# ManuelZ/image-search-engine

Measured on AMD Instinct MI355X. Metric: queries/sec, exact brute-force L2 kNN (recall@10 vs exact CPU), 1Mx512 fp32 index, k=10, higher is better.
Workload: dtype f32; 1 GPU; 1000000x512 fp32 uniform[0,1) index (default_rng 1234), L2, k=10, nq=16 queries per step, index resident in HBM, steps issued round-robin on 16 HIP streams; 400 untimed steps ahead of the warm-up bring the GPU out of its idle power state; n=1000000, d=512, k=10, nq=16

## Files before the change

image-search-engine_amd/_native.py:

```python
from __future__ import annotations

import ctypes
import os

import torch

_HERE = os.path.dirname(os.path.abspath(__file__))
LIB_PATH = os.environ.get("ISE_KNN_LIB") or os.path.join(_HERE, "csrc", "libise_knn.so")

METRIC_INNER_PRODUCT = 0
METRIC_L2 = 1
MAX_K = 2048
STORE_F32, STORE_BF16 = 0, 1

E_INVALID, E_HIP, E_NOMEM, E_NODEVICE = -1, -2, -3, -4

_f32p = ctypes.POINTER(ctypes.c_float)
_i64p = ctypes.POINTER(ctypes.c_int64)
_u64p = ctypes.POINTER(ctypes.c_uint64)
_vp = ctypes.c_void_p
_i64 = ctypes.c_int64
_int = ctypes.c_int
PROTOTYPES = [
    ("ise_version", _int, []),
# ... 13 lines not shown
    ("ise_index_add_host", _int, [_vp, _vp, _i64]),
    ("ise_index_add_device", _int, [_vp, _vp, _i64, _vp]),
    ("ise_index_reconstruct_host", _int, [_vp, _i64, _i64, _vp]),
    ("ise_index_search_host", _int, [_vp, _vp, _i64, _int, _vp, _vp]),
    ("ise_index_search_device", _int, [_vp, _vp, _i64, _int, _vp, _vp, _vp]),
    ("ise_index_search_keys_device", _int, [_vp, _vp, _i64, _int, ctypes.c_uint32, _vp, _vp]),
    ("ise_index_assign_device", _int, [_vp, _vp, _i64, _vp, _vp, _vp]),
    ("ise_merge_keys_device", _int, [_vp, _int, _i64, _int, _int, _vp, _vp, _int, _vp]),
    ("ise_normalize_rows_device", _int, [_vp, _i64, _int, _int, _vp]),
    ("ise_normalize_rows_host", _int, [_vp, _i64, _int, _int]),
    ("ise_bovw_histogram_device", _int, [_vp, _vp, _i64, _int, _vp, _int, _vp]),
    ("ise_index_short_stats", _int, [_vp, _vp]),
    ("ise_index_half_stats", _int, [_vp, _u64p]),
    ("ise_index_shadow_row", _int, [_vp, _i64, _f32p]),
    ("ise_index_byte_stats", _int, [_vp, _u64p]),
    ("ise_index_byte_row", _int, [_vp, _i64, _f32p]),
    ("ise_index_stage_query_debug", _int, [_vp, _vp, _int, _vp, _i64, _f32p, ctypes.POINTER(ctypes.c_int32)]),
    ("ise_index_range_search_host", _int, [_vp, _vp, _i64, ctypes.c_float, ctypes.POINTER(_vp)]),
    ("ise_range_result_get", _int, [_vp, _i64p, ctypes.POINTER(_vp), ctypes.POINTER(_vp), ctypes.POINTER(_vp)]),
    ("ise_range_result_destroy", _int, [_vp]),
    ("ise_index_range_stats", _int, [_vp, _u64p]),
    ("ise_index_remove_ids_host", _int, [_vp, _vp, _i64, _i64p]),
    ("ise_index_remove_range", _int, [_vp, _i64, _i64, _i64p]),
    ("ise_index_remove_stats", _int, [_vp, _u64p]),
    ("ise_index_remove_last_timing", _int, [_vp, _f32p, _u64p]),
    ("ise_selector_create_range", _int, [_vp, _i64, _i64, ctypes.POINTER(_vp)]),
    ("ise_selector_create_ids", _int, [_vp, _vp, _i64, _int, ctypes.POINTER(_vp)]),
    ("ise_selector_create_bitmap", _int, [_vp, _vp, _i64, ctypes.POINTER(_vp)]),
    ("ise_selector_info", _int, [_vp, _i64p]),
    ("ise_selector_destroy", _int, [_vp]),
# ... 69 lines not shown
```

image-search-engine_amd/csrc/ise_knn.hip:

```cpp

#include "ise_common.hpp"
#include "ise_scan_params.hpp"
#include "ise_assign.hpp"
#include "ise_exact.hpp"
#include "ise_merge.hpp"
#include "ise_exact_scan.hpp"
#include "ise_gemm_scan.hpp"
#include "ise_gemm_bf16.hpp"
#include "ise_rows.hpp"
#include "ise_short_scan.hpp"
#include "ise_range.hpp"
#include "ise_sel_scan.hpp"
#include "ise_stage.hpp"
#include "ise_remove.hpp"

static thread_local std::string g_err;
static int fail(int code, const std::string& msg) {
    g_err = msg;
    return code;
}
int ise_fail_(int code, const std::string& msg) { return fail(code, msg); }
#define HIP_TRY(expr)                                                                      \
    do {                                                                                   \
        hipError_t e_ = (expr);                                                            \
// ... 12 lines not shown
    bool shift_pinned = false;
    long long mu_rows = 0;
    long long norms_rows = 0;
    void* xh = nullptr;
    float* hmeta = nullptr;
    int dph = 0;
    bool shadow_off = false;
    void* xq8 = nullptr;
    uint32_t* bmeta = nullptr;
    int dpb = 0;
    bool byte_off = false;
    double byte_rel = 0.0;
    double byte_rho = 1.0;
    unsigned long long half_batches = 0;
    unsigned long long byte_batches = 0;
    unsigned long long* stats_dev = nullptr;
    unsigned long long mu_updates = 0;
    unsigned long long gemm_chunks = 0;
    struct WorkSlot {
        u64* part = nullptr;
        size_t part_elems = 0;
        u64* keys_tmp = nullptr;
        size_t keys_tmp_elems = 0;
        u64* xchg = nullptr;
        size_t xchg_elems = 0;
        uint32_t xchg_seq = 0;
        char* gemm = nullptr;
        size_t gemm_bytes = 0;
        u64* fl_state = nullptr;
        int* fl_list = nullptr;
// ... 627 lines not shown
    else if (uses_shift(h)) ise_launch_short_f32_shift(ch, waves, bpc, grid, lds, st, sp, tp);
    else ise_launch_short_f32_plain(ch, waves, bpc, grid, lds, st, sp, tp);
}

struct ScanPlan {
    int nblocks, tiles_total, tiles_per_block, nqt, ch, kpass, kb, waves, T;
    size_t lds;
    bool exact;
    int kc;
    bool gemm;
    size_t gemm_bytes;
    bool half;
    bool byte;
    bool short_;
    int short_bpc;
};

static void launch_scan(const ise_index* h, const ScanPlan& pl, dim3 grid, hipStream_t st, const ScanParams& sp) {
    const int ch = pl.ch, waves = pl.waves, T = pl.T;
    const size_t lds = pl.lds;
    if (pl.byte) ise_launch_scan_i8_shadow(ch, waves, T, grid, lds, st, sp);
    else if (pl.half) ise_launch_scan_f16_shadow(ch, waves, T, grid, lds, st, sp);
    else if (h->storage == ISE_STORE_BF16) ise_launch_scan_bf16(ch, waves, T, grid, lds, st, sp);
    else if (uses_shift(h)) ise_launch_scan_f32_shift(ch, waves, T, grid, lds, st, sp);
    else ise_launch_scan_f32_plain(ch, waves, T, grid, lds, st, sp);
}

static int exact_extra(int k) {
    static const int forced = [] { const char* e = getenv("ISE_EXACT_EXTRA"); return e ? atoi(e) : 0; }();
    (void)k;
// ... 2 lines not shown
static float exact_beta(const ise_index* h) { return (0.5625f * h->dp + 256.f) * 5.9604645e-8f * 1.02f; }
static float half_beta(const ise_index* h) { return (5.f * h->dph + 128.f) * 5.9604645e-8f * 1.02f; }
static float half_lo_shrink(const ise_index* h) { return 1.f - ((float)h->dp / 16.f + 96.f) * 5.9604645e-8f; }
static float byte_beta(const ise_index* h) { return ((float)h->dp / 8.f + 64.f) * 5.9604645e-8f * 1.02f; }
struct EnvKnobs {
    std::atomic<int> force_exact{0};
    std::atomic<int> no_direct{0};
    std::atomic<int> no_short{0};
    std::atomic<int> short_tpb_max{0};
    std::atomic<int> direct_short_max_tiles{0};
    std::atomic<int> range_stage_cap{0};
    std::atomic<int> no_half{0};
    std::atomic<int> no_byte{0};
    std::atomic<int> fail_byte_alloc{0};
    std::atomic<int> remove_slab_rows{0};
    void refresh() {
        auto flag = [](const char* name) { const char* e = getenv(name); return (e && e[0] == '1') ? 1 : 0; };
        auto num = [](const char* name) { const char* e = getenv(name); return e ? atoi(e) : 0; };
        force_exact.store(flag("ISE_FORCE_EXACT"));
        no_direct.store(flag("ISE_NO_DIRECT"));
        no_short.store(flag("ISE_NO_SHORT"));
        short_tpb_max.store(num("ISE_SHORT_TPB_MAX"));
        direct_short_max_tiles.store(num("ISE_DIRECT_SHORT_MAX_TILES"));
        range_stage_cap.store(num("ISE_RANGE_STAGE_CAP"));
        no_half.store(flag("ISE_NO_HALF_FILTER"));
        no_byte.store(flag("ISE_NO_BYTE_FILTER"));
        fail_byte_alloc.store(flag("ISE_FAIL_BYTE_ALLOC"));
        remove_slab_rows.store(num("ISE_REMOVE_SLAB_ROWS"));
    }
};
static EnvKnobs& knobs() {
    static EnvKnobs k;
    static std::once_flag once;
    std::call_once(once, [] { k.refresh(); });
    return k;
}
extern "C" int ise_refresh_env_knobs(void) {
    knobs().refresh();
    return ISE_OK;
}
int ise_remove_slab_rows_() { return knobs().remove_slab_rows.load(std::memory_order_relaxed); }
static bool force_exact() { return knobs().force_exact.load(std::memory_order_relaxed) != 0; }
static bool byte_alloc_refused() { return knobs().fail_byte_alloc.load(std::memory_order_relaxed) != 0; }

static bool xchg_enabled() {
    static const bool on = [] { const char* e = getenv("ISE_NO_XCHG"); return !(e && e[0] == '1'); }();
    return on;
}

static int make_plan(const ise_index* h, long long nq, int k, ScanPlan* pl, bool allow_short = true,
                     bool allow_half = true) {
    pl->exact = uses_shift(h);
    const bool shadow_ok = allow_half && pl->exact && h->xh != nullptr && !knobs().no_half.load(std::memory_order_relaxed);
    pl->byte = shadow_ok && h->xq8 != nullptr && byte_rel_ok(h) && !knobs().no_byte.load(std::memory_order_relaxed) &&
               k <= BYTE_MAX_K && nq <= BYTE_MAX_NQ;
    pl->kc = pl->exact ? (pl->byte ? BYTE_KC : k + exact_extra(k)) : k;
    pl->kpass = pl->kc < KPASS_MAX ? pl->kc : KPASS_MAX;
    pl->kb = pl->kpass <= 16 ? 16 : (pl->kpass <= 32 ? 32 : KB_MAX);
    pl->half = shadow_ok && (pl->byte || pl->kc <= SHADOW_MAX_KC);
    const size_t rb = pl->byte ? byte_row_bytes(h) : (pl->half ? shadow_row_bytes(h) : row_bytes(h));
    auto lds_bytes = [&](int waves, int T) {
        if (pl->byte) return scan_lds_layout(qs_stride_byte(h), waves, T, pl->kb, true, scan_seeded_boot(true, waves, T));
        return pl->half ? scan_lds_layout(qs_stride_half(h), waves, T, pl->kb, true) : scan_lds_bytes(h, waves, T, pl->kb);
    };
    pl->ch = chunk_steps_rb(rb);
#ifdef ISE_ABLATE
// ... 27 lines not shown
        if (!wv) break;
        const double cost = (double)((nq + 16 * t - 1) / (16 * t)) * pass_cost[t];
        if (!pl->T || cost < best - 1e-9) {
            pl->T = t;
            pl->waves = wv;
            pl->lds = lds;
            best = cost;
        }
    }
    if (!pl->T) return fail(ISE_E_INVALID, "d too large: a 16-query tile must fit the 160 KiB LDS "
                                              "(float32 rows: d <= 2240, bf16 rows: d <= 4480)");
    if ((pl->T == 1 || pl->waves == 16) && pl->ch > 4) pl->ch = 4;
    pl->tiles_total = (int)((h->n + 15) / 16);
    int blocks_per_cu = (pl->T == 1 && pl->waves <= 8 && pl->lds <= LDS_LIMIT / 2) ? 2 : 1;
#ifdef ISE_ABLATE
    if (const char* e = getenv("ISE_PLAN")) {
        int wv = 8, bpc = 2;
        if (pl->T == 1 && sscanf(e, "%d,%d", &wv, &bpc) == 2 && (wv == 4 || wv == 8) && bpc >= 1) {
            pl->waves = wv;
            pl->lds = lds_bytes(wv, 1);
            blocks_per_cu = bpc;
        }
    }
#endif
    const bool long_rows = rb > 2048;
    const int nqt_plan = (int)((nq + 16 * pl->T - 1) / (16 * pl->T));
    const int min_tiles = (int)std::max<size_t>(1, 65536 / (16 * rb));
    const int slots = h->num_cu * blocks_per_cu;
    const int nb_packed = std::min(slots, (pl->tiles_total + pl->waves - 1) / pl->waves);
    const int nb_spread = std::min(std::max(1, slots / nqt_plan), (pl->tiles_total + min_tiles - 1) / min_tiles);
    int nb = std::max(nb_packed, nb_spread);
    if (nb < 1) nb = 1;
    if (nb > MERGE_LISTS_MAX) nb = MERGE_LISTS_MAX;
    pl->tiles_per_block = (pl->tiles_total + nb - 1) / nb;
    if (pl->tiles_per_block < 1) pl->tiles_per_block = 1;
    pl->nblocks = (pl->tiles_total + pl->tiles_per_block - 1) / pl->tiles_per_block;
    if (pl->nblocks < 1) pl->nblocks = 1;
    if (long_rows && pl->T == 1 && pl->waves <= 8 && pl->tiles_per_block <= pl->waves && chunk_steps_rb(rb) == 8) pl->ch = 8;
    pl->nqt = (int)((nq + 16 * pl->T - 1) / (16 * pl->T));
    pl->gemm = false;
    pl->gemm_bytes = 0;
    pl->short_ = false;
    pl->short_bpc = 0;
    static const bool short_t2 = [] { const char* e = getenv("ISE_SHORT_T2"); return !(e && e[0] == '0'); }();
    const int short_T = nq <= 16 ? 1 : 2;
    if (allow_short && !pl->byte && (nq <= 16 || (short_t2 && nq <= 64)) && pl->kc <= pl->kpass && h->n > 0 &&
        !knobs().no_short.load(std::memory_order_relaxed)) {
        int tpb_max = knobs().short_tpb_max.load(std::memory_order_relaxed);
        if (tpb_max <= 0 || tpb_max > SHORT_TPB_MAX) tpb_max = SHORT_TPB_MAX;
        const int S = qs_stride_for(h);
        static const int shapes[2][3] = {{16, 1, 1}, {8, 2, 1}};
        int first = row_bytes(h) <= 2048 ? 0 : 2;
#ifdef ISE_ABLATE
        if (const char* e = getenv("ISE_SHORT_SHAPE")) first = std::max(first, std::min(1, atoi(e)));
#endif
        for (int si = first; si < 2 && !pl->short_; si++) {
            const int wv = shapes[si][0], bpc = shapes[si][1];
            const int short_nqt = (int)((nq + 16 * short_T - 1) / (16 * short_T));
            const int packed = (pl->tiles_total + wv - 1) / wv;
            const int spread = std::min(std::max(1, h->num_cu * bpc / short_nqt), (pl->tiles_total + min_tiles - 1) / min_tiles);
            int nbs = std::max(1, std::min(h->num_cu * bpc * shapes[si][2], std::max(packed, spread)));
            nbs = std::min(nbs, MERGE_LISTS_MAX);
            const int tpb = (pl->tiles_total + nbs - 1) / nbs;
            const size_t lds = short_lds_layout(S, tpb, wv, short_T);
            if (tpb <= tpb_max && lds <= (size_t)LDS_LIMIT / bpc) {
                pl->short_ = true;
                pl->nblocks = nbs;
                pl->tiles_per_block = tpb;
                pl->lds = lds;
                pl->waves = wv;
                pl->short_bpc = bpc;
                pl->T = short_T;
                pl->nqt = short_nqt;
                pl->ch = std::min(chunk_steps(h), 4);
                pl->half = false;
                pl->byte = false;
            }
        }
    }
    return ISE_OK;
}

static int ensure_workspace(ise_index::WorkSlot* w, const ScanPlan& pl, long long nq, bool* changed) {
    if (!w->done) HIP_TRY(hipEventCreateWithFlags(&w->done, hipEventDisableTiming));
    const size_t need = std::max<size_t>((size_t)pl.nqt * pl.nblocks * (16 * pl.T) * pl.kpass, (size_t)MERGE_LISTS_MAX * XPASS_MAX);
    if (need > w->part_elems) {
        if (w->part) (void)hipFree(w->part);
        w->part = nullptr;
        w->part_elems = 0;
        HIP_TRY(hipMalloc(&w->part, need * sizeof(u64)));
        w->part_elems = need;
        *changed = true;
    }
    const size_t needx = (size_t)pl.nqt * (16 * pl.T) * pl.nblocks;
    if (needx > w->xchg_elems) {
        if (w->xchg) (void)hipFree(w->xchg);
        w->xchg = nullptr;
        w->xchg_elems = 0;
        HIP_TRY(hipMalloc(&w->xchg, needx * sizeof(u64)));
        HIP_TRY(hipMemset(w->xchg, 0xFF, needx * sizeof(u64)));
        w->xchg_elems = needx;
        w->xchg_seq = 0;
        if (const char* e = getenv("ISE_XCHG_SEQ_START"))
            w->xchg_seq = (uint32_t)strtoul(e, nullptr, 0);
        *changed = true;
    }
    if (pl.kc > pl.kpass) {
        const size_t need2 = (size_t)nq * ((size_t)pl.kc + 2 + pl.kpass + XPASS_MAX);
        if (need2 > w->keys_tmp_elems) {
// ... 89 lines not shown
    *seq = ++w->fl_seq;
    return ISE_OK;
}

template <bool RERANK>
static void launch_merge(unsigned grid, size_t lds, hipStream_t st, const MergeParams& mp, const ExactParams& xp) {
    hipLaunchKernelGGL((merge_kernel<RERANK>), dim3(grid), dim3(MERGE_THREADS), lds, st, mp, xp);
}

static int enqueue_exact_fallback(ise_index* h, ise_index::WorkSlot* w, const ScanPlan& pl, const ExactParams& xp,
                                  long long nq, hipStream_t st) {
    ExactScanParams xs;
    xs.xb = (const float*)h->xb; xs.q = xp.q; xs.n = h->n; xs.d = h->d; xs.dp = h->dp;
    xs.id_base = xp.id_base; xs.fl_state = w->fl_state; xs.fl_list = w->fl_list; xs.seq = xp.seq;
    xs.part = w->part;
    xs.rows_per_block = (long long)pl.tiles_per_block * 16;
    xs.arrive = reinterpret_cast<unsigned int*>(w->fl_state + 1);
    xs.direct_n = 0;
    const size_t lds = (size_t)XQ * h->dp * 4 + (size_t)XQ * 4 * 32 * 8;
    MergeParams mp;
    mp.lists = w->part; mp.qt = 1; mp.n_lists = pl.nblocks; mp.nq = (int)nq; mp.metric = h->metric;
    mp.fl_state = w->fl_state; mp.fl_list = w->fl_list; mp.seq = xp.seq; mp.dbg = nullptr; mp.gate = nullptr;
    const int k = xp.k;
    if (k <= XPASS_MAX) {
        xs.kpass = k; xs.floor_keys = nullptr;
        mp.k = k; mp.stride_list = k; mp.stride_qtile = (long long)pl.nblocks * k;
        mp.D = xp.D; mp.I = xp.I; mp.keys_out = xp.keys_out; mp.out_by_pos = 0;
        hipLaunchKernelGGL(exact_scan_kernel<XQ>, dim3((unsigned)pl.nblocks), dim3(256), lds, st, xs, mp);
        HIP_TRY(hipGetLastError());
        return ISE_OK;
    }
    u64* fb_floor = w->keys_tmp + (size_t)nq * ((size_t)pl.kc + 1 + pl.kpass);
    u64* fb_pass = fb_floor + nq;
    const int kp = XPASS_MAX;
    for (int off = 0; off < k; off += kp) {
        xs.kpass = kp; xs.floor_keys = off ? fb_floor : nullptr;
        mp.k = kp; mp.stride_list = kp; mp.stride_qtile = (long long)pl.nblocks * kp;
        mp.D = nullptr; mp.I = nullptr; mp.keys_out = fb_pass; mp.out_by_pos = 1;
        hipLaunchKernelGGL(exact_scan_kernel<XQ>, dim3((unsigned)pl.nblocks), dim3(256), lds, st, xs, mp);
        const long long tot = nq * kp;
        hipLaunchKernelGGL(exact_scatter_kernel, dim3((unsigned)((tot + 255) / 256)), dim3(256), 0, st, xp,
                           (const u64*)fb_pass, kp, off, fb_floor);
        HIP_TRY(hipGetLastError());
    }
    return ISE_OK;
}

static bool no_direct() { return knobs().no_direct.load(std::memory_order_relaxed) != 0; }
static bool direct_applies(const ise_index* h, const ise_index::WorkSlot* w, const ScanPlan& pl, long long nq, int k,
                           int* blocks_out) {
    if (!pl.exact || nq != 1 || k > XPASS_MAX || h->n <= 0 || !w->fl_state || no_direct() || force_exact()) return false;
    int max_tiles = knobs().direct_short_max_tiles.load(std::memory_order_relaxed);
    if (max_tiles <= 0) max_tiles = 128;
    if (pl.short_ && pl.tiles_total > max_tiles) return false;
// ... 55 lines not shown
    GemmLayout g;
    size_t o = 0;
    auto take = [&](size_t bytes) { const size_t at = o; o += (bytes + 255) / 256 * 256; return at; };
    g.qprep = take((size_t)GEMM_NQ_MAX * qs_stride_for(h) * 4);
    g.xn = take((size_t)GEMM_NQ_MAX * 4);
    g.tau = take((size_t)GEMM_NQ_MAX * 4);
    g.ccnt = take((size_t)(GEMM_NQ_MAX * GEMM_SUBS + 64) * 4);
    g.dump = take((size_t)GEMM_NQ_MAX * GEMM_SAMPLE_SLABS * 128 * 4);
    g.cand = take((size_t)GEMM_NQ_MAX * GEMM_CAPQ * 8);
    g.wbuf = take((size_t)h->num_cu * 8 * GEMM_CAPW * 16);
    g.wcnt = take((size_t)h->num_cu * 8 * 4);
    g.total = o;
    return g;
}

static int plan_for_batch(const ise_index* h, long long nq, int k, ScanPlan* pl) {
    const bool big = gemm_applies(h, nq, k);
    int rc = make_plan(h, big ? std::min<long long>(nq, GEMM_NQ_MAX) : nq, k, pl);
    if (rc) return rc;
    pl->gemm = big;
    pl->gemm_bytes = big ? gemm_layout(h).total : 0;
    return ISE_OK;
}

template <int NS, bool DUMP, bool IPM>
static void launch_gemm_metric(int grid, size_t lds, hipStream_t st, const GemmScanParams& gp) {
    static LdsAttrOnce attr;
    attr.ensure(reinterpret_cast<const void*>(&gemm_scan_kernel<NS, DUMP, IPM>), LDS_LIMIT);
    hipLaunchKernelGGL((gemm_scan_kernel<NS, DUMP, IPM>), dim3(grid), dim3(512), lds, st, gp);
}
template <int NS, bool DUMP>
static void launch_gemm_one(int grid, size_t lds, hipStream_t st, const GemmScanParams& gp) {
    if (gp.metric == ISE_METRIC_INNER_PRODUCT) launch_gemm_metric<NS, DUMP, true>(grid, lds, st, gp);
// ... 86 lines not shown
                             int k, uint32_t id_base, float* D_dev, long long* I_dev, u64* keys_out, hipStream_t st,
                             TimedOut* tm, const unsigned int* gate) {
    int rc;
    ScanParams sp;
    sp.xb = h->xb; sp.norms = h->norms; sp.q = q_dev; sp.mu = h->mu; sp.floor_keys = nullptr; sp.part = w->part;
    sp.n = h->n; sp.d = h->d; sp.dp = h->dp; sp.qs_stride = qs_stride_for(h);
    sp.row_slots = (int)(row_bytes(h) / 16);
    sp.nq = (int)nq; sp.k = pl.kpass; sp.kb = pl.kb; sp.metric = h->metric; sp.id_base = id_base;
    sp.beta = pl.exact ? exact_beta(h) : 0.f;
    if (pl.byte) {
        sp.xb = h->xq8; sp.bmeta = h->bmeta;
        sp.qs_stride = qs_stride_byte(h); sp.row_slots = (int)(byte_row_bytes(h) / 16);
        sp.beta = byte_beta(h); sp.lo_shrink = half_lo_shrink(h);
        h->half_batches++;
        h->byte_batches++;
    } else if (pl.half) {
        sp.xb = h->xh; sp.norms = h->hmeta; sp.herr = h->hmeta + h->cap; sp.hexp = h->hmeta + 2 * h->cap;
        sp.qs_stride = qs_stride_half(h); sp.row_slots = (int)(shadow_row_bytes(h) / 16);
        sp.beta = half_beta(h); sp.lo_shrink = half_lo_shrink(h);
        h->half_batches++;
    }
    sp.tiles_total = pl.tiles_total; sp.tiles_per_block = pl.tiles_per_block;
    sp.xchg = xchg_enabled() ? w->xchg : nullptr;
    sp.xchg_seq = 0;
    sp.gate = gate;
    sp.ablate = 0;
    sp.stamps = nullptr;
#ifdef ISE_ABLATE
    if (const char* e = getenv("ISE_ABLATE")) sp.ablate = atoi(e);
    if (const char* e = getenv("ISE_STAMPS")) sp.stamps = (unsigned long long*)strtoull(e, nullptr, 0);
// ... 246 lines not shown
                       keys_out);
    HIP_TRY(hipGetLastError());
    ScanPlan pl;
    rc = make_plan(h, nq, k, &pl, false);
    if (rc) return rc;
    rc = scan_path_enqueue(h, w, pl, q_dev, nq, k, id_base, D_dev, I_dev, keys_out, st, nullptr, rerun);
    if (rc) return rc;
    if (tm && tm->on) HIP_TRY(hipEventRecord(tm->e2, st));
    return ISE_OK;
}

static int search_enqueue(ise_index* h, const float* q_dev, long long nq, int k, uint32_t id_base, float* D_dev,
                          long long* I_dev, u64* keys_out, hipStream_t st, TimedOut* tm) {
    int rc = prepare_shift_locked(h, st);
    if (rc) return rc;
    ScanPlan pl;
    rc = plan_for_batch(h, nq, k, &pl);
    if (rc) return rc;
    rc = ensure_workspaces(h, pl, pl.gemm ? std::min<long long>(nq, GEMM_NQ_MAX) : nq);
    if (rc) return rc;
    ise_index::WorkSlot* w = nullptr;
    bool same_stream = false;
    for (auto& s : h->ws)
        if (s.used && s.last_stream == st) { w = &s; same_stream = true; break; }
    if (!w)
        for (auto& s : h->ws)
            if (!s.used) { w = &s; break; }
    if (!w) w = &h->ws[h->ws_next++ % ise_index::NWS];
    if (w->used && !same_stream) HIP_TRY(hipStreamWaitEvent(st, w->done, 0));
    struct Release {
        ise_index::WorkSlot* w;
        hipStream_t st;
// ... 1047 lines not shown
extern "C" int ise_index_range_stats(ise_index_t* h, uint64_t* out2) {
    if (!h || !out2) return fail(ISE_E_INVALID, "NULL argument");
    std::lock_guard<std::mutex> lk(h->rg_mu);
    out2[0] = h->range_batches;
    out2[1] = h->range_overflows;
    return ISE_OK;
}

extern "C" int ise_index_short_stats(ise_index_t* h, uint64_t* out1) {
    if (!h || !out1) return fail(ISE_E_INVALID, "NULL argument");
    std::lock_guard<std::mutex> lk(h->mu_);
    out1[0] = h->short_batches;
    return ISE_OK;
}

extern "C" int ise_index_half_stats(ise_index_t* h, uint64_t* out1) {
    if (!h || !out1) return fail(ISE_E_INVALID, "NULL argument");
    std::lock_guard<std::mutex> lk(h->mu_);
    out1[0] = h->half_batches;
    return ISE_OK;
}

extern "C" int ise_index_byte_stats(ise_index_t* h, uint64_t* out2) {
    if (!h || !out2) return fail(ISE_E_INVALID, "NULL argument");
    std::lock_guard<std::mutex> lk(h->mu_);
    out2[0] = h->byte_batches;
    out2[1] = (h->xq8 && byte_rel_ok(h)) ? 1 : 0;
    return ISE_OK;
}

// ... 253 lines not shown
```

image-search-engine_amd/csrc/ise_scan.hpp:

```cpp
#pragma once
#include "ise_common.hpp"
#include "ise_scan_params.hpp"
#include "ise_select.hpp"
#include "ise_stage.hpp"

#ifndef ISE_FINAL_FILTER
#define ISE_FINAL_FILTER 1
#endif

#ifdef ISE_ABLATE
#define ABL(bit) (p.ablate & (bit))
#define STAMP(i)                                                                                   \
    do {                                                                                           \
        if (p.stamps && lane == 0)                                                                 \
            p.stamps[((size_t)blockIdx.x * W + w) * 16 + (i)] = __builtin_amdgcn_s_memrealtime();  \
    } while (0)
#define CSTAMP(i)                                                                                  \
    do {                                                                                           \
        if (p.stamps && lane == 0)                                                                 \
            p.stamps[((size_t)blockIdx.x * W + w) * 16 + (i)] = __builtin_amdgcn_s_memtime();      \
    } while (0)
#else
#define ABL(bit) 0
#define STAMP(i) do {} while (0)
#define CSTAMP(i) do {} while (0)
#endif

template <int CH, int W, int T, bool BF16, bool SHIFT, int RM = ROWS_OWN>
__global__ __launch_bounds__(W * 64, T == 1 ? W / 2 : (W / 4 > 0 ? W / 4 : 1)) void scan_kernel(const ScanParams p) {
    constexpr bool HALF = RM == ROWS_F16, BYTE = RM == ROWS_I8, SHADOW = HALF || BYTE;
    static_assert(!(BF16 && SHIFT), "the shift is applied to fp32 rows only");
    static_assert(!SHADOW || SHIFT, "shadow rows belong to float32 L2 indexes");
    constexpr bool F32S = SHIFT && !SHADOW;
    if (p.gate && *p.gate == 0u) return;
    constexpr int BLOCK_THREADS = W * 64;
    constexpr bool XCHG = T >= 3 || (T == 2 && W == 8) || (RM == ROWS_I8 && T == 1 && W == 8);
    constexpr bool FFILT = XCHG && ISE_FINAL_FILTER;
    constexpr bool NBOOT = scan_seeded_boot(RM == ROWS_I8, W, T);
    static_assert(!NBOOT || XCHG, "the seeded boot reads the exchange");
    constexpr int NQ = 16 * T;
    constexpr int TPR = W >= 16 ? 32 : BLOCK_THREADS / 16;
    constexpr int KPLB = (W * 16 + 63) / 64;
    constexpr int KPLF = (KB_MAX + W * CAP + 63) / 64;
    static_assert(KB_MAX + CAP <= 64 && MERGE_TRIG + 4 <= CAP, "list sizes");
    extern __shared__ __align__(16) unsigned char smem[];
    const int S = p.qs_stride;
    const int kb = p.kb;
    float* mus = reinterpret_cast<float*>(smem);
    float* qs = mus + S;
    float* xn = qs + NQ * S;
    float* xe = xn + NQ;
    int* xsh = reinterpret_cast<int*>(xe + NQ);
    u64* tauS = reinterpret_cast<u64*>(xn + (SHADOW ? 3 : 1) * NQ);
// ... 465 lines not shown
        for (int b = 31; b >= 0; b--) {
            const uint32_t hm = b == 31 ? 0u : 0xFFFFFFFFu << (b + 1);
            auto zero_here = [&](uint32_t v) { return ((v ^ prefix) & hm) == 0u && ((v >> b) & 1u) == 0u; };
            const int c0 = __popcll(__ballot(zero_here(v0))) + __popcll(__ballot(zero_here(v1))) +
                           __popcll(__ballot(zero_here(v2))) + __popcll(__ballot(zero_here(v3)));
            if (rank > c0) {
                rank -= c0;
                prefix |= 1u << b;
            }
        }
        return prefix;
    };
    constexpr bool XFOLD = NBOOT;
    constexpr int XE = 4;
    constexpr int XGRID = 512;
    auto xchg_request = [&](int qq, int half, u64(&e)[XE]) {
        const int nb = (int)gridDim.x;
        const int G = (nb + 255) >> 8;
        const u64* src = p.xchg + ((size_t)blockIdx.y * NQ + qq) * nb;
#pragma unroll
        for (int i = 0; i < XE; i++) {
            const int idx = (lane + 64 * (2 * half + (i >> 1))) * G + (i & 1);
            e[i] = __hip_atomic_load(src + (((i & 1) < G && idx < nb) ? idx : 0), __ATOMIC_RELAXED, __HIP_MEMORY_SCOPE_AGENT);
        }
    };
    auto xchg_fold = [&](int half, const u64(&e)[XE], uint32_t best) -> uint32_t {
        const int nb = (int)gridDim.x;
        const int G = (nb + 255) >> 8;
#pragma unroll
        for (int i = 0; i < XE; i++) {
            const int idx = (lane + 64 * (2 * half + (i >> 1))) * G + (i & 1);
            if ((i & 1) < G && idx < nb && (uint32_t)(e[i] >> 32) == p.xchg_seq) best = min(best, (uint32_t)e[i]);
        }
        return best;
    };
    auto lanes_kth = [&](uint32_t v) -> uint32_t {
        uint32_t prefix = 0;
        int rank = k;
        for (int b = 31; b >= 0; b--) {
            const uint32_t hm = b == 31 ? 0u : 0xFFFFFFFFu << (b + 1);
            const int c0 = __popcll(__ballot(((v ^ prefix) & hm) == 0u && ((v >> b) & 1u) == 0u));
            if (rank > c0) {
                rank -= c0;
                prefix |= 1u << b;
            }
        }
        return prefix;
    };
    auto exchange = [&]() {
        STAMP(12);
        for (int qq = w; qq < NQ; qq += W) {
            uint32_t prefix;
            if (XFOLD && (int)gridDim.x <= XGRID && !ABL(16384)) {
                u64 e[XE];
                xchg_request(qq, 0, e);
                const uint32_t b0 = xchg_fold(0, e, 0xFFFFFFFFu);
                xchg_request(qq, 1, e);
                prefix = lanes_kth(xchg_fold(1, e, b0));
            } else {
                prefix = xchg_prefix(qq);
            }
            if (prefix != 0xFFFFFFFFu) {
                const u64 bound = ((u64)prefix << 32) | 0xFFFFFFFFull;
                if (FFILT && lane == (qq - w) / W) xbound = bound;
                if (lane == 0) {
                    while (atomicCAS(&lockS[qq], 0, 1) != 0) __builtin_amdgcn_s_sleep(1);
                }
                wave_lds_fence();
                if (lane == 0 && bound < tauS[qq]) tauS[qq] = bound;
                wave_lds_fence();
                if (lane == 0) atomicExch(&lockS[qq], 0);
            }
        }
// ... 1 lines not shown
    };

    auto seed_phase = [&]() {
        STAMP(10);
        u64 xe_[XE];
        xchg_request(w, 0, xe_);
        __syncthreads();
        STAMP(11);
        const u64 lt_mask = (1ull << lane) - 1ull;
        for (int qq = w; qq < NQ; qq += W) {
            u64 kk[4];
#pragma unroll
            for (int e = 0; e < 4; e++)
                kk[e] = ((e < 2 ? boot : home2) + (size_t)qq * (W * 16))[lane + 64 * (e & 1)];
            uint32_t folded = xchg_fold(0, xe_, 0xFFFFFFFFu);
            xchg_request(qq, 1, xe_);
            folded = xchg_fold(1, xe_, folded);
            if (qq + W < NQ) xchg_request(qq + W, 0, xe_);
            const uint32_t prefix = lanes_kth(folded);
            if (qq == w) STAMP(12);
            const u64 bound = ((u64)prefix << 32) | 0xFFFFFFFFull;
            if (FFILT && prefix != 0xFFFFFFFFu && lane == (qq - w) / W) xbound = bound;
            u64 keep[4];
            int n_in = 0;
#pragma unroll
            for (int e = 0; e < 4; e++) {
                keep[e] = __ballot(kk[e] <= bound && kk[e] != KEY_PAD);
                n_in += __popcll(keep[e]);
            }
            if (prefix != 0xFFFFFFFFu && n_in <= kb) {
                int off = 0;
#pragma unroll
                for (int e = 0; e < 4; e++) {
                    if ((keep[e] >> lane) & 1ull) bootw[qq * kb + off + __popcll(keep[e] & lt_mask)] = kk[e];
// ... 165 lines not shown
```

image-search-engine_amd/csrc/ise_scan_launch.hpp:

```cpp
#pragma once
#include "ise_scan.hpp"

template <int CH, int W, int T, bool BF16, bool SHIFT, int RM>
static void launch_one(dim3 grid, size_t lds, hipStream_t st, const ScanParams& sp) {
    static LdsAttrOnce attr;
    attr.ensure(reinterpret_cast<const void*>(&scan_kernel<CH, W, T, BF16, SHIFT, RM>), LDS_LIMIT);
    hipLaunchKernelGGL((scan_kernel<CH, W, T, BF16, SHIFT, RM>), grid, dim3(W * 64), lds, st, sp);
}
template <int W, int T, bool BF16, bool SHIFT, int RM>
static void launch_scan_ch(int ch, dim3 grid, size_t lds, hipStream_t st, const ScanParams& sp) {
    switch (ch) {
        case 8:
            if constexpr (W < 16) launch_one<8, W, T, BF16, SHIFT, RM>(grid, lds, st, sp);
            else launch_one<4, W, T, BF16, SHIFT, RM>(grid, lds, st, sp);
            break;
        case 4: launch_one<4, W, T, BF16, SHIFT, RM>(grid, lds, st, sp); break;
        case 2: launch_one<2, W, T, BF16, SHIFT, RM>(grid, lds, st, sp); break;
        default: launch_one<1, W, T, BF16, SHIFT, RM>(grid, lds, st, sp); break;
    }
}
template <bool BF16, bool SHIFT, int RM = ROWS_OWN>
static void launch_scan_v(int ch, int waves, int T, dim3 grid, size_t lds, hipStream_t st, const ScanParams& sp) {
    if constexpr (RM == ROWS_I8) {
        if (waves == 4) launch_scan_ch<4, 1, BF16, SHIFT, RM>(ch, grid, lds, st, sp);
        else launch_scan_ch<8, 1, BF16, SHIFT, RM>(ch, grid, lds, st, sp);
    } else if (T == 1 && waves == 4) launch_scan_ch<4, 1, BF16, SHIFT, RM>(ch, grid, lds, st, sp);
    else if (T == 1) launch_scan_ch<8, 1, BF16, SHIFT, RM>(ch, grid, lds, st, sp);
    else if (T == 2 && waves == 16) launch_scan_ch<16, 2, BF16, SHIFT, RM>(ch, grid, lds, st, sp);
    else if (T == 2) launch_scan_ch<8, 2, BF16, SHIFT, RM>(ch, grid, lds, st, sp);
    else if (T == 3) launch_scan_ch<8, 3, BF16, SHIFT, RM>(ch, grid, lds, st, sp);
    else if constexpr (BF16) launch_scan_ch<8, 4, true, false, ROWS_OWN>(ch, grid, lds, st, sp);
}
```

image-search-engine_amd/csrc/ise_scan_params.hpp:

```cpp
#pragma once
#include "ise_common.hpp"

enum RowMode : int { ROWS_OWN = 0, ROWS_F16 = 1, ROWS_I8 = 2 };

struct ScanParams {
    const void* xb;
    const float* norms;
    const float* herr = nullptr;
    const float* hexp = nullptr;
    const uint32_t* bmeta = nullptr;
    const float* q;
    const float* mu;
    const u64* floor_keys;
    u64* part;
    long long n;
    int d, dp, qs_stride;
    int row_slots;
    int nq, k, kb, metric;
    uint32_t id_base;
    float beta;
    float lo_shrink = 1.f;
    int tiles_total, tiles_per_block;
    unsigned long long* xchg;
    uint32_t xchg_seq;
// ... 31 lines not shown
```

image-search-engine_amd/faiss_compat.py:

```python
from __future__ import annotations

import ctypes
import struct
import threading

import numpy as np

from . import _native as _n

METRIC_INNER_PRODUCT = _n.METRIC_INNER_PRODUCT
METRIC_L2 = _n.METRIC_L2

_FLT_MAX = float(np.finfo(np.float32).max)


def _as_rows(x, d=None) -> np.ndarray:
    x = np.ascontiguousarray(np.asarray(x), dtype=np.float32)
    assert x.ndim == 2, "expected a 2-D array"
    if d is not None:
        assert x.shape[1] == d, f"dimension mismatch: got {x.shape[1]}, index has d={d}"
    return x


def _default_device() -> int:
# ... 214 lines not shown

    def short_stats(self) -> dict:
        out = (ctypes.c_uint64 * 1)()
        _n.check(_n.lib.ise_index_short_stats(self._h, out))
        return {"short_batches": int(out[0])}

    def half_stats(self) -> dict:
        out = (ctypes.c_uint64 * 1)()
        _n.check(_n.lib.ise_index_half_stats(self._h, out))
        return {"half_batches": int(out[0])}

    def byte_stats(self) -> dict:
        out = (ctypes.c_uint64 * 2)()
        _n.check(_n.lib.ise_index_byte_stats(self._h, out))
        return {"byte_batches": int(out[0]), "byte_route": bool(out[1])}

    def byte_row(self, i: int) -> tuple:
        out = (ctypes.c_float * 2)()
        _n.check(_n.lib.ise_index_byte_row(self._h, int(i), out))
        return float(out[0]), float(out[1])

    def shadow_row(self, i: int) -> tuple:
        out = (ctypes.c_float * 3)()
        _n.check(_n.lib.ise_index_shadow_row(self._h, int(i), out))
        return float(out[0]), float(out[1]), int(out[2])

    def stage_query_debug(self, q: "torch.Tensor", route: str) -> dict:
        import torch
        assert q.is_cuda and q.dtype == torch.float32 and q.dim() == 1 and q.is_contiguous() and q.numel() == self.d
        es = {"half": 2, "byte": 1}[route]
# ... 829 lines not shown
```

include/ise_knn.h:

```cpp
#ifndef ISE_KNN_H
#define ISE_KNN_H

#include <stdint.h>

#ifdef __cplusplus
extern "C" {
#endif

#define ISE_METRIC_INNER_PRODUCT 0
#define ISE_METRIC_L2 1

#define ISE_STORE_F32 0
#define ISE_STORE_BF16 1

#define ISE_OK 0
#define ISE_E_INVALID -1
#define ISE_E_HIP -2
#define ISE_E_NOMEM -3
#define ISE_E_NODEVICE -4

#define ISE_MAX_K 2048

typedef struct ise_index ise_index_t;

// ... 8 lines not shown
int ise_index_reset(ise_index_t* h);
int ise_index_info(const ise_index_t* h, int* d, int* metric, int64_t* ntotal, int* device);

int ise_index_add_host(ise_index_t* h, const float* x, int64_t n);
int ise_index_add_device(ise_index_t* h, const float* x_dev, int64_t n, void* stream);

int ise_index_set_shift(ise_index_t* h, const float* mu_host);
int ise_index_get_shift(ise_index_t* h, float* mu_host);

int ise_index_stats(ise_index_t* h, uint64_t* out4);

int ise_index_short_stats(ise_index_t* h, uint64_t* out1);

int ise_index_half_stats(ise_index_t* h, uint64_t* out1);
int ise_index_byte_stats(ise_index_t* h, uint64_t* out2);
int ise_index_shadow_row(ise_index_t* h, int64_t i, float* out3);
int ise_index_byte_row(ise_index_t* h, int64_t i, float* out2);

int ise_index_stage_query_debug(ise_index_t* h, const void* q_dev, int route, void* limbs, int64_t limbs_bytes,
                                float* out2, int32_t* info3);

int ise_refresh_env_knobs(void);

int ise_index_reserve_workspaces(ise_index_t* h, int64_t nq, int k);

int ise_index_reconstruct_host(ise_index_t* h, int64_t i0, int64_t n, float* out);

int ise_index_search_host(ise_index_t* h, const float* q, int64_t nq, int k,
                          float* D, int64_t* I);
int ise_index_host_stats(ise_index_t* h, uint64_t* out3);
// ... 100 lines not shown
```

Measured before the change: 167,000 queries/s.

## Shrink byte-scan grid when batches arrive on alternating streams

Adds a "depth" plan. When consecutive searches come from different streams, the byte-filter scan launches half as many blocks, each covering more tiles, so concurrent batches from several streams can share the CUs. It also adds a single-request exchange variant (ROWS_I8_ONE) for grids of at most 256 blocks, which folds the cross-block k-th bound from one load round instead of two. Workspaces and the fallback exact path keep the isolated block count. The risk is lower per-batch parallelism if streams do not actually overlap.

After: 174,400 queries/s, median of 6. 4.4% higher.

```diff
diff --git a/image-search-engine_amd/_native.py b/image-search-engine_amd/_native.py
--- a/image-search-engine_amd/_native.py
+++ b/image-search-engine_amd/_native.py
@@ -51,6 +51,7 @@
     ("ise_index_half_stats", _int, [_vp, _u64p]),
     ("ise_index_shadow_row", _int, [_vp, _i64, _f32p]),
     ("ise_index_byte_stats", _int, [_vp, _u64p]),
+    ("ise_index_depth_stats", _int, [_vp, _u64p]),
     ("ise_index_byte_row", _int, [_vp, _i64, _f32p]),
     ("ise_index_stage_query_debug", _int, [_vp, _vp, _int, _vp, _i64, _f32p, ctypes.POINTER(ctypes.c_int32)]),
     ("ise_index_range_search_host", _int, [_vp, _vp, _i64, ctypes.c_float, ctypes.POINTER(_vp)]),
diff --git a/image-search-engine_amd/csrc/ise_knn.hip b/image-search-engine_amd/csrc/ise_knn.hip
--- a/image-search-engine_amd/csrc/ise_knn.hip
+++ b/image-search-engine_amd/csrc/ise_knn.hip
@@ -50,6 +50,9 @@
     double byte_rho = 1.0;
     unsigned long long half_batches = 0;
     unsigned long long byte_batches = 0;
+    unsigned long long byte_deep_batches = 0;
+    hipStream_t prev_stream = nullptr;
+    bool prev_search = false;
     unsigned long long* stats_dev = nullptr;
     unsigned long long mu_updates = 0;
     unsigned long long gemm_chunks = 0;
@@ -707,6 +710,7 @@
     bool byte;
     bool short_;
     int short_bpc;
+    int depth, fb_nblocks, fb_tiles_per_block;
 };
 
 static void launch_scan(const ise_index* h, const ScanPlan& pl, dim3 grid, hipStream_t st, const ScanParams& sp) {
@@ -739,6 +743,7 @@
     std::atomic<int> no_byte{0};
     std::atomic<int> fail_byte_alloc{0};
     std::atomic<int> remove_slab_rows{0};
+    std::atomic<int> scan_depth{0};
     void refresh() {
         auto flag = [](const char* name) { const char* e = getenv(name); return (e && e[0] == '1') ? 1 : 0; };
         auto num = [](const char* name) { const char* e = getenv(name); return e ? atoi(e) : 0; };
@@ -752,6 +757,7 @@
         no_byte.store(flag("ISE_NO_BYTE_FILTER"));
         fail_byte_alloc.store(flag("ISE_FAIL_BYTE_ALLOC"));
         remove_slab_rows.store(num("ISE_REMOVE_SLAB_ROWS"));
+        scan_depth.store(std::max(0, num("ISE_SCAN_DEPTH")));
     }
 };
 static EnvKnobs& knobs() {
@@ -774,7 +780,7 @@
 }
 
 static int make_plan(const ise_index* h, long long nq, int k, ScanPlan* pl, bool allow_short = true,
-                     bool allow_half = true) {
+                     bool allow_half = true, int depth = 1) {
     pl->exact = uses_shift(h);
     const bool shadow_ok = allow_half && pl->exact && h->xh != nullptr && !knobs().no_half.load(std::memory_order_relaxed);
     pl->byte = shadow_ok && h->xq8 != nullptr && byte_rel_ok(h) && !knobs().no_byte.load(std::memory_order_relaxed) &&
@@ -832,19 +838,25 @@
     pl->tiles_total = (int)((h->n + 15) / 16);
     int blocks_per_cu = (pl->T == 1 && pl->waves <= 8 && pl->lds <= LDS_LIMIT / 2) ? 2 : 1;
 #ifdef ISE_ABLATE
+    int slot_div = 1;
     if (const char* e = getenv("ISE_PLAN")) {
-        int wv = 8, bpc = 2;
-        if (pl->T == 1 && sscanf(e, "%d,%d", &wv, &bpc) == 2 && (wv == 4 || wv == 8) && bpc >= 1) {
+        int wv = 8, bpc = 2, div = 1;
+        if (pl->T == 1 && sscanf(e, "%d,%d,%d", &wv, &bpc, &div) >= 2 && (wv == 4 || wv == 8) && bpc >= 1 && div >= 1) {
             pl->waves = wv;
             pl->lds = lds_bytes(wv, 1);
             blocks_per_cu = bpc;
+            slot_div = div;
         }
     }
 #endif
     const bool long_rows = rb > 2048;
     const int nqt_plan = (int)((nq + 16 * pl->T - 1) / (16 * pl->T));
     const int min_tiles = (int)std::max<size_t>(1, 65536 / (16 * rb));
+#ifdef ISE_ABLATE
+    const int slots = std::max(1, h->num_cu * blocks_per_cu / slot_div);
+#else
     const int slots = h->num_cu * blocks_per_cu;
+#endif
     const int nb_packed = std::min(slots, (pl->tiles_total + pl->waves - 1) / pl->waves);
     const int nb_spread = std::min(std::max(1, slots / nqt_plan), (pl->tiles_total + min_tiles - 1) / min_tiles);
     int nb = std::max(nb_packed, nb_spread);
@@ -854,6 +866,19 @@
     if (pl->tiles_per_block < 1) pl->tiles_per_block = 1;
     pl->nblocks = (pl->tiles_total + pl->tiles_per_block - 1) / pl->tiles_per_block;
     if (pl->nblocks < 1) pl->nblocks = 1;
+    pl->depth = 1;
+    pl->fb_nblocks = pl->nblocks;
+    pl->fb_tiles_per_block = pl->tiles_per_block;
+    if (depth > 1 && pl->byte && pl->T == 1 && pl->waves == 8 && nb == slots && nb_packed == slots && slots / depth >= 1) {
+        const int nbd = slots / depth;
+        const int tpb = (pl->tiles_total + nbd - 1) / nbd;
+        if (tpb >= 55) {
+            pl->depth = depth;
+            pl->tiles_per_block = tpb;
+            pl->nblocks = (pl->tiles_total + tpb - 1) / tpb;
+        }
+    }
+    if (pl->nblocks > pl->fb_nblocks) return fail(ISE_E_INVALID, "internal: the deep plan has more blocks than the isolated one");
     if (long_rows && pl->T == 1 && pl->waves <= 8 && pl->tiles_per_block <= pl->waves && chunk_steps_rb(rb) == 8) pl->ch = 8;
     pl->nqt = (int)((nq + 16 * pl->T - 1) / (16 * pl->T));
     pl->gemm = false;
@@ -883,8 +908,8 @@
             const size_t lds = short_lds_layout(S, tpb, wv, short_T);
             if (tpb <= tpb_max && lds <= (size_t)LDS_LIMIT / bpc) {
                 pl->short_ = true;
-                pl->nblocks = nbs;
-                pl->tiles_per_block = tpb;
+                pl->nblocks = pl->fb_nblocks = nbs;
+                pl->tiles_per_block = pl->fb_tiles_per_block = tpb;
                 pl->lds = lds;
                 pl->waves = wv;
                 pl->short_bpc = bpc;
@@ -901,7 +926,7 @@
 
 static int ensure_workspace(ise_index::WorkSlot* w, const ScanPlan& pl, long long nq, bool* changed) {
     if (!w->done) HIP_TRY(hipEventCreateWithFlags(&w->done, hipEventDisableTiming));
-    const size_t need = std::max<size_t>((size_t)pl.nqt * pl.nblocks * (16 * pl.T) * pl.kpass, (size_t)MERGE_LISTS_MAX * XPASS_MAX);
+    const size_t need = std::max<size_t>((size_t)pl.nqt * pl.fb_nblocks * (16 * pl.T) * pl.kpass, (size_t)MERGE_LISTS_MAX * XPASS_MAX);
     if (need > w->part_elems) {
         if (w->part) (void)hipFree(w->part);
         w->part = nullptr;
@@ -910,7 +935,7 @@
         w->part_elems = need;
         *changed = true;
     }
-    const size_t needx = (size_t)pl.nqt * (16 * pl.T) * pl.nblocks;
+    const size_t needx = (size_t)pl.nqt * (16 * pl.T) * pl.fb_nblocks;
     if (needx > w->xchg_elems) {
         if (w->xchg) (void)hipFree(w->xchg);
         w->xchg = nullptr;
@@ -1030,19 +1055,19 @@
     xs.xb = (const float*)h->xb; xs.q = xp.q; xs.n = h->n; xs.d = h->d; xs.dp = h->dp;
     xs.id_base = xp.id_base; xs.fl_state = w->fl_state; xs.fl_list = w->fl_list; xs.seq = xp.seq;
     xs.part = w->part;
-    xs.rows_per_block = (long long)pl.tiles_per_block * 16;
+    xs.rows_per_block = (long long)pl.fb_tiles_per_block * 16;
     xs.arrive = reinterpret_cast<unsigned int*>(w->fl_state + 1);
     xs.direct_n = 0;
     const size_t lds = (size_t)XQ * h->dp * 4 + (size_t)XQ * 4 * 32 * 8;
     MergeParams mp;
-    mp.lists = w->part; mp.qt = 1; mp.n_lists = pl.nblocks; mp.nq = (int)nq; mp.metric = h->metric;
+    mp.lists = w->part; mp.qt = 1; mp.n_lists = pl.fb_nblocks; mp.nq = (int)nq; mp.metric = h->metric;
     mp.fl_state = w->fl_state; mp.fl_list = w->fl_list; mp.seq = xp.seq; mp.dbg = nullptr; mp.gate = nullptr;
     const int k = xp.k;
     if (k <= XPASS_MAX) {
         xs.kpass = k; xs.floor_keys = nullptr;
-        mp.k = k; mp.stride_list = k; mp.stride_qtile = (long long)pl.nblocks * k;
+        mp.k = k; mp.stride_list = k; mp.stride_qtile = (long long)pl.fb_nblocks * k;
         mp.D = xp.D; mp.I = xp.I; mp.keys_out = xp.keys_out; mp.out_by_pos = 0;
-        hipLaunchKernelGGL(exact_scan_kernel<XQ>, dim3((unsigned)pl.nblocks), dim3(256), lds, st, xs, mp);
+        hipLaunchKernelGGL(exact_scan_kernel<XQ>, dim3((unsigned)pl.fb_nblocks), dim3(256), lds, st, xs, mp);
         HIP_TRY(hipGetLastError());
         return ISE_OK;
     }
@@ -1051,9 +1076,9 @@
     const int kp = XPASS_MAX;
     for (int off = 0; off < k; off += kp) {
         xs.kpass = kp; xs.floor_keys = off ? fb_floor : nullptr;
-        mp.k = kp; mp.stride_list = kp; mp.stride_qtile = (long long)pl.nblocks * kp;
+        mp.k = kp; mp.stride_list = kp; mp.stride_qtile = (long long)pl.fb_nblocks * kp;
         mp.D = nullptr; mp.I = nullptr; mp.keys_out = fb_pass; mp.out_by_pos = 1;
-        hipLaunchKernelGGL(exact_scan_kernel<XQ>, dim3((unsigned)pl.nblocks), dim3(256), lds, st, xs, mp);
+        hipLaunchKernelGGL(exact_scan_kernel<XQ>, dim3((unsigned)pl.fb_nblocks), dim3(256), lds, st, xs, mp);
         const long long tot = nq * kp;
         hipLaunchKernelGGL(exact_scatter_kernel, dim3((unsigned)((tot + 255) / 256)), dim3(256), 0, st, xp,
                            (const u64*)fb_pass, kp, off, fb_floor);
@@ -1139,9 +1164,9 @@
     return g;
 }
 
-static int plan_for_batch(const ise_index* h, long long nq, int k, ScanPlan* pl) {
+static int plan_for_batch(const ise_index* h, long long nq, int k, ScanPlan* pl, int depth = 1) {
     const bool big = gemm_applies(h, nq, k);
-    int rc = make_plan(h, big ? std::min<long long>(nq, GEMM_NQ_MAX) : nq, k, pl);
+    int rc = make_plan(h, big ? std::min<long long>(nq, GEMM_NQ_MAX) : nq, k, pl, true, true, depth);
     if (rc) return rc;
     pl->gemm = big;
     pl->gemm_bytes = big ? gemm_layout(h).total : 0;
@@ -1258,6 +1283,7 @@
         sp.beta = byte_beta(h); sp.lo_shrink = half_lo_shrink(h);
         h->half_batches++;
         h->byte_batches++;
+        if (pl.depth > 1) h->byte_deep_batches++;
     } else if (pl.half) {
         sp.xb = h->xh; sp.norms = h->hmeta; sp.herr = h->hmeta + h->cap; sp.hexp = h->hmeta + 2 * h->cap;
         sp.qs_stride = qs_stride_half(h); sp.row_slots = (int)(shadow_row_bytes(h) / 16);
@@ -1534,8 +1560,12 @@
                           long long* I_dev, u64* keys_out, hipStream_t st, TimedOut* tm) {
     int rc = prepare_shift_locked(h, st);
     if (rc) return rc;
+    int depth = knobs().scan_depth.load(std::memory_order_relaxed);
+    if (depth <= 0) depth = (h->prev_search && h->prev_stream != st) ? 2 : 1;
+    h->prev_search = true;
+    h->prev_stream = st;
     ScanPlan pl;
-    rc = plan_for_batch(h, nq, k, &pl);
+    rc = plan_for_batch(h, nq, k, &pl, depth);
     if (rc) return rc;
     rc = ensure_workspaces(h, pl, pl.gemm ? std::min<long long>(nq, GEMM_NQ_MAX) : nq);
     if (rc) return rc;
@@ -2613,6 +2643,14 @@
     return ISE_OK;
 }
 
+extern "C" int ise_index_depth_stats(ise_index_t* h, uint64_t* out2) {
+    if (!h || !out2) return fail(ISE_E_INVALID, "NULL argument");
+    std::lock_guard<std::mutex> lk(h->mu_);
+    out2[0] = h->byte_batches - h->byte_deep_batches;
+    out2[1] = h->byte_deep_batches;
+    return ISE_OK;
+}
+
 extern "C" int ise_index_half_stats(ise_index_t* h, uint64_t* out1) {
     if (!h || !out1) return fail(ISE_E_INVALID, "NULL argument");
     std::lock_guard<std::mutex> lk(h->mu_);
diff --git a/image-search-engine_amd/csrc/ise_scan.hpp b/image-search-engine_amd/csrc/ise_scan.hpp
--- a/image-search-engine_amd/csrc/ise_scan.hpp
+++ b/image-search-engine_amd/csrc/ise_scan.hpp
@@ -28,15 +28,15 @@
 
 template <int CH, int W, int T, bool BF16, bool SHIFT, int RM = ROWS_OWN>
 __global__ __launch_bounds__(W * 64, T == 1 ? W / 2 : (W / 4 > 0 ? W / 4 : 1)) void scan_kernel(const ScanParams p) {
-    constexpr bool HALF = RM == ROWS_F16, BYTE = RM == ROWS_I8, SHADOW = HALF || BYTE;
+    constexpr bool HALF = RM == ROWS_F16, BYTE = RM == ROWS_I8 || RM == ROWS_I8_ONE, SHADOW = HALF || BYTE;
     static_assert(!(BF16 && SHIFT), "the shift is applied to fp32 rows only");
     static_assert(!SHADOW || SHIFT, "shadow rows belong to float32 L2 indexes");
     constexpr bool F32S = SHIFT && !SHADOW;
     if (p.gate && *p.gate == 0u) return;
     constexpr int BLOCK_THREADS = W * 64;
-    constexpr bool XCHG = T >= 3 || (T == 2 && W == 8) || (RM == ROWS_I8 && T == 1 && W == 8);
+    constexpr bool XCHG = T >= 3 || (T == 2 && W == 8) || (BYTE && T == 1 && W == 8);
     constexpr bool FFILT = XCHG && ISE_FINAL_FILTER;
-    constexpr bool NBOOT = scan_seeded_boot(RM == ROWS_I8, W, T);
+    constexpr bool NBOOT = scan_seeded_boot(BYTE, W, T);
     static_assert(!NBOOT || XCHG, "the seeded boot reads the exchange");
     constexpr int NQ = 16 * T;
     constexpr int TPR = W >= 16 ? 32 : BLOCK_THREADS / 16;
@@ -532,23 +532,24 @@
     constexpr bool XFOLD = NBOOT;
     constexpr int XE = 4;
     constexpr int XGRID = 512;
+    constexpr bool XREQ1 = RM == ROWS_I8_ONE;
     auto xchg_request = [&](int qq, int half, u64(&e)[XE]) {
         const int nb = (int)gridDim.x;
-        const int G = (nb + 255) >> 8;
+        const int G = XREQ1 ? 1 : (nb + 255) >> 8;
         const u64* src = p.xchg + ((size_t)blockIdx.y * NQ + qq) * nb;
 #pragma unroll
         for (int i = 0; i < XE; i++) {
-            const int idx = (lane + 64 * (2 * half + (i >> 1))) * G + (i & 1);
-            e[i] = __hip_atomic_load(src + (((i & 1) < G && idx < nb) ? idx : 0), __ATOMIC_RELAXED, __HIP_MEMORY_SCOPE_AGENT);
+            const int idx = XREQ1 ? lane + 64 * i : (lane + 64 * (2 * half + (i >> 1))) * G + (i & 1);
+            e[i] = __hip_atomic_load(src + (((XREQ1 || (i & 1) < G) && idx < nb) ? idx : 0), __ATOMIC_RELAXED, __HIP_MEMORY_SCOPE_AGENT);
         }
     };
     auto xchg_fold = [&](int half, const u64(&e)[XE], uint32_t best) -> uint32_t {
         const int nb = (int)gridDim.x;
-        const int G = (nb + 255) >> 8;
+        const int G = XREQ1 ? 1 : (nb + 255) >> 8;
 #pragma unroll
         for (int i = 0; i < XE; i++) {
-            const int idx = (lane + 64 * (2 * half + (i >> 1))) * G + (i & 1);
-            if ((i & 1) < G && idx < nb && (uint32_t)(e[i] >> 32) == p.xchg_seq) best = min(best, (uint32_t)e[i]);
+            const int idx = XREQ1 ? lane + 64 * i : (lane + 64 * (2 * half + (i >> 1))) * G + (i & 1);
+            if ((XREQ1 || (i & 1) < G) && idx < nb && (uint32_t)(e[i] >> 32) == p.xchg_seq) best = min(best, (uint32_t)e[i]);
         }
         return best;
     };
@@ -565,6 +566,26 @@
         }
         return prefix;
     };
+    auto lanes_kth4 = [&](const u64(&e)[XE]) -> uint32_t {
+        const int nb = (int)gridDim.x;
+        uint32_t v[XE];
+#pragma unroll
+        for (int i = 0; i < XE; i++)
+            v[i] = (lane + 64 * i < nb && (uint32_t)(e[i] >> 32) == p.xchg_seq) ? (uint32_t)e[i] : 0xFFFFFFFFu;
+        uint32_t prefix = 0;
+        int rank = k;
+        for (int b = 31; b >= 0; b--) {
+            const uint32_t hm = b == 31 ? 0u : 0xFFFFFFFFu << (b + 1);
+            int c0 = 0;
+#pragma unroll
+            for (int i = 0; i < XE; i++) c0 += __popcll(__ballot(((v[i] ^ prefix) & hm) == 0u && ((v[i] >> b) & 1u) == 0u));
+            if (rank > c0) {
+                rank -= c0;
+                prefix |= 1u << b;
+            }
+        }
+        return prefix;
+    };
     auto exchange = [&]() {
         STAMP(12);
         for (int qq = w; qq < NQ; qq += W) {
@@ -572,9 +593,12 @@
             if (XFOLD && (int)gridDim.x <= XGRID && !ABL(16384)) {
                 u64 e[XE];
                 xchg_request(qq, 0, e);
-                const uint32_t b0 = xchg_fold(0, e, 0xFFFFFFFFu);
-                xchg_request(qq, 1, e);
-                prefix = lanes_kth(xchg_fold(1, e, b0));
+                uint32_t folded = xchg_fold(0, e, 0xFFFFFFFFu);
+                if constexpr (!XREQ1) {
+                    xchg_request(qq, 1, e);
+                    folded = xchg_fold(1, e, folded);
+                }
+                prefix = lanes_kth(folded);
             } else {
                 prefix = xchg_prefix(qq);
             }
@@ -606,10 +630,13 @@
             for (int e = 0; e < 4; e++)
                 kk[e] = ((e < 2 ? boot : home2) + (size_t)qq * (W * 16))[lane + 64 * (e & 1)];
             uint32_t folded = xchg_fold(0, xe_, 0xFFFFFFFFu);
-            xchg_request(qq, 1, xe_);
-            folded = xchg_fold(1, xe_, folded);
+            if constexpr (!XREQ1) {
+                xchg_request(qq, 1, xe_);
+                folded = xchg_fold(1, xe_, folded);
+            }
+            const uint32_t all4 = (XREQ1 && ABL(32768)) ? lanes_kth4(xe_) : 0u;
             if (qq + W < NQ) xchg_request(qq + W, 0, xe_);
-            const uint32_t prefix = lanes_kth(folded);
+            const uint32_t prefix = (XREQ1 && ABL(32768)) ? all4 : lanes_kth(folded);
             if (qq == w) STAMP(12);
             const u64 bound = ((u64)prefix << 32) | 0xFFFFFFFFull;
             if (FFILT && prefix != 0xFFFFFFFFu && lane == (qq - w) / W) xbound = bound;
diff --git a/image-search-engine_amd/csrc/ise_scan_launch.hpp b/image-search-engine_amd/csrc/ise_scan_launch.hpp
--- a/image-search-engine_amd/csrc/ise_scan_launch.hpp
+++ b/image-search-engine_amd/csrc/ise_scan_launch.hpp
@@ -23,6 +23,7 @@
 static void launch_scan_v(int ch, int waves, int T, dim3 grid, size_t lds, hipStream_t st, const ScanParams& sp) {
     if constexpr (RM == ROWS_I8) {
         if (waves == 4) launch_scan_ch<4, 1, BF16, SHIFT, RM>(ch, grid, lds, st, sp);
+        else if (grid.x <= 256) launch_scan_ch<8, 1, BF16, SHIFT, ROWS_I8_ONE>(ch, grid, lds, st, sp);
         else launch_scan_ch<8, 1, BF16, SHIFT, RM>(ch, grid, lds, st, sp);
     } else if (T == 1 && waves == 4) launch_scan_ch<4, 1, BF16, SHIFT, RM>(ch, grid, lds, st, sp);
     else if (T == 1) launch_scan_ch<8, 1, BF16, SHIFT, RM>(ch, grid, lds, st, sp);
diff --git a/image-search-engine_amd/csrc/ise_scan_params.hpp b/image-search-engine_amd/csrc/ise_scan_params.hpp
--- a/image-search-engine_amd/csrc/ise_scan_params.hpp
+++ b/image-search-engine_amd/csrc/ise_scan_params.hpp
@@ -1,7 +1,7 @@
 #pragma once
 #include "ise_common.hpp"
 
-enum RowMode : int { ROWS_OWN = 0, ROWS_F16 = 1, ROWS_I8 = 2 };
+enum RowMode : int { ROWS_OWN = 0, ROWS_F16 = 1, ROWS_I8 = 2, ROWS_I8_ONE = 3 };
 
 struct ScanParams {
     const void* xb;
diff --git a/image-search-engine_amd/faiss_compat.py b/image-search-engine_amd/faiss_compat.py
--- a/image-search-engine_amd/faiss_compat.py
+++ b/image-search-engine_amd/faiss_compat.py
@@ -252,6 +252,11 @@
         out = (ctypes.c_uint64 * 2)()
         _n.check(_n.lib.ise_index_byte_stats(self._h, out))
         return {"byte_batches": int(out[0]), "byte_route": bool(out[1])}
+
+    def depth_stats(self) -> dict:
+        out = (ctypes.c_uint64 * 2)()
+        _n.check(_n.lib.ise_index_depth_stats(self._h, out))
+        return {"isolated_batches": int(out[0]), "deep_batches": int(out[1])}
 
     def byte_row(self, i: int) -> tuple:
         out = (ctypes.c_float * 2)()
diff --git a/include/ise_knn.h b/include/ise_knn.h
--- a/include/ise_knn.h
+++ b/include/ise_knn.h
@@ -46,6 +46,7 @@
 
 int ise_index_half_stats(ise_index_t* h, uint64_t* out1);
 int ise_index_byte_stats(ise_index_t* h, uint64_t* out2);
+int ise_index_depth_stats(ise_index_t* h, uint64_t* out2);
 int ise_index_shadow_row(ise_index_t* h, int64_t i, float* out3);
 int ise_index_byte_row(ise_index_t* h, int64_t i, float* out2);
 
```
